# NikolasMarkou/blind_image_denoising

Measured on AMD Instinct MI355X. Metric: denoised images/sec (256x256x3) + MAE vs ref, resnet_1x18, higher is better.
Workload: dtype f16x2 split (hi+lo, fp32 accumulate)

## Files before the change

blind_image_denoising_amd/csrc/fused_h3w.hip:

```cpp
#include "h3v_core.h"
#include "h3_bands.h"
#include "base_rows.h"

#ifndef H3W_PRIO_SET
#define H3W_PRIO_SET 0
#endif
#if H3W_PRIO_SET == 1
#define H3W_PRIO_A1 0
#define H3W_PRIO_B1 1
#define H3W_PRIO_A2 2
#define H3W_PRIO_B2 3
#elif H3W_PRIO_SET == 2
#define H3W_PRIO_A1 3
#define H3W_PRIO_B1 2
#define H3W_PRIO_A2 1
#define H3W_PRIO_B2 0
#elif H3W_PRIO_SET == 3
#define H3W_PRIO_A1 0
#define H3W_PRIO_B1 2
#define H3W_PRIO_A2 0
#define H3W_PRIO_B2 2
#elif H3W_PRIO_SET == 4
#define H3W_PRIO_A1 2
#define H3W_PRIO_B1 0
#define H3W_PRIO_A2 2
#define H3W_PRIO_B2 0
#endif
#ifndef H3W_PRIO_A1
#define H3W_PRIO_A1 1
#endif
#ifndef H3W_PRIO_B1
#define H3W_PRIO_B1 1
#endif
#ifndef H3W_PRIO_A2
#define H3W_PRIO_A2 1
#endif
#ifndef H3W_PRIO_B2
#define H3W_PRIO_B2 1
#endif

#ifndef H3W_XCD_ORDER
#define H3W_XCD_ORDER 1
#endif

struct H3WGeom {
    static constexpr int NG = 9, GW = 16 * NG;
    static constexpr int G = 3;
    static constexpr int NR = 3, NW = 12, NT = 768;
    static constexpr int SW = 128;
    static constexpr int PITCH = (GW + 2) * 16;
    static constexpr int NRX0 = 5, NRM = 2, NRX1 = 3, NRO = 2;
    static constexpr int PD = 3;
    static constexpr int UNROLL = 6;
    static constexpr int X0_PLANE = (NRX0 * PITCH + 255) / 256 * 256, M_PLANE = (NRM * PITCH + 255) / 256 * 256;
    static constexpr int X1_PLANE = (NRX1 * PITCH + 255) / 256 * 256;
    static constexpr int OUT_PLANE = GW * 16, OUT_SLOT = 4 * OUT_PLANE;
    static constexpr int X0_OFF = 0, M1_OFF = X0_OFF + 4 * X0_PLANE, X1_OFF = M1_OFF + 4 * M_PLANE, M2_OFF = X1_OFF + 4 * X1_PLANE;
    static constexpr int OUT_OFF = M2_OFF + 4 * M_PLANE, LDS_BYTES = OUT_OFF + NRO * OUT_SLOT;
    static constexpr int BIN_RING = 4, BIN_ROWPX = GW + 4;
    static constexpr int BIN_SLOT = 2 * BIN_ROWPX * 8;
    static constexpr int BIN_OFF = LDS_BYTES, BWA_OFF = BIN_OFF + BIN_RING * BIN_SLOT, BINVS_OFF = BWA_OFF + 3 * 64 * 16;
    static constexpr int BRED_OFF = BINVS_OFF + 16, LDS_BYTES_BASE = BRED_OFF + NT * 4;
    static_assert(LDS_BYTES_BASE <= 160 * 1024 && BIN_OFF % 16 == 0 && BIN_SLOT % 16 == 0 && LDS_BYTES_BASE % 16 == 0, "LDS (producer)");
    static constexpr int LEAD = 12;
    static constexpr int NSTAMP = 4;
    static_assert(UNROLL % NRM == 0 && UNROLL % NRO == 0 && UNROLL % NRX1 == 0 && UNROLL % 3 == 0, "static slots");
    static_assert(NRX0 == PD + 2, "x0 ring: rows s-1 (residual), s (conv1a), s+1 (landed), s+2, s+3 (in flight)");
    static_assert(LDS_BYTES <= 160 * 1024, "LDS");
    static_assert(3 * X0_PLANE + NRX0 * PITCH < 65536, "fragment offsets fit the 16-bit ds offset");
};

struct H3WTile : BandUnit {
    int X0, X1;
    int G0;
    int D0, D1;
};

__device__ __forceinline__ H3WTile h3w_tile(const FusedH3WArgs& a, const int t)
{
    H3WTile r{bf_band_unit<H3W_XCD_ORDER != 0>(a, t)};
    r.X0 = r.sx * H3WGeom::SW;
    r.X1 = min(a.W, r.X0 + H3WGeom::SW);
    r.G0 = min(max(r.X0 - 8, 0), max(a.W - H3WGeom::GW, 0));
    r.D0 = max(0, (r.X0 - 4) & ~7);
    r.D1 = min(a.W, (r.X1 + 4 + 7) & ~7);
    return r;
}

template <int INP>
struct H3WRoleA {
    using Gm = H3WGeom;
    const char* tin;
    char* tmid;
    h8 w[13];
    f32x4 acc[Gm::G][3];
    int rp, rs;
    int wr;
    float inv_s, relu_floor;
    float lane_scale[Gm::G];
    bool skip_last = false;

    __device__ __forceinline__ void init(const void* wimg, const FusedH3WArgs& a, const float* aux, const int lane, const int gc0)
    {
        const int q = lane >> 4;
#pragma unroll
        for (int i = 0; i < 13; ++i) w[i] = reinterpret_cast<const h8*>(wimg)[bf_band_wimage(a, i) * 64 + lane];
        inv_s = aux[0];
        relu_floor = a.act1_relu ? 0.f : -__builtin_inff();
        rp = (q & 1) * INP + (gc0 + (q >> 1)) * 16;
        rs = ((q & 1) + 2 * (q >> 1)) * INP + (gc0 + 2) * 16;
        wr = (q >> 1) * Gm::M_PLANE + (gc0 + 1) * 16 + (q & 1) * 8;
#pragma unroll
        for (int g = 0; g < Gm::G; ++g)
#pragma unroll
            for (int k = 0; k < 3; ++k) acc[g][k] = (f32x4){0.f, 0.f, 0.f, 0.f};
    }
    __device__ __forceinline__ void set_tile(const H3WTile& t, const int W, const int gc0)
    {
#pragma unroll
        for (int g = 0; g < Gm::G; ++g) lane_scale[g] = (t.G0 + gc0 + 16 * g < W) ? inv_s : 0.f;
    }

    __device__ __forceinline__ H3VFrag load(const int islot_bytes, const int g) const
    {
        H3VFrag f;
        const char* p = tin + rp + islot_bytes;
        f.ph = *reinterpret_cast<const h8*>(p + g * 256);
        f.pl = *reinterpret_cast<const h8*>(p + g * 256 + 2 * INP);
        f.s = *reinterpret_cast<const h8*>(tin + rs + islot_bytes + g * 256);
        return f;
    }

    __device__ __forceinline__ H3VEpi<true> epilogue(const int g, const int mslot, const f32x4 v, const bool rowok) const
    {
        H3VEpi<true> e;
        e.v = v;
        e.sc = rowok ? lane_scale[g] : 0.f;
        e.floor_ = relu_floor;
        e.p = tmid + wr + mslot * Gm::PITCH + g * 256;
        e.lo_off = 2 * Gm::M_PLANE;
        return e;
    }

    template <int J, class Epi>
    __device__ __forceinline__ void mfmas(const int g, const int a1, const int a2, const H3VFrag& cur, f32x4& c0, Epi* epi)
    {
        if constexpr (J < 15) {
            constexpr int k = J / 3, which = J % 3;
            if (!(H3V_ABLATE & 8) && !(skip_last && g == Gm::G - 1)) {
                if constexpr (which == 0) acc[g][a2] = h3v_mfma(cur, w, 2, k, acc[g][a2]);
                else if constexpr (which == 1) acc[g][a1] = h3v_mfma(cur, w, 1, k, acc[g][a1]);
                else c0 = h3v_mfma(cur, w, 0, k, c0);
            } else if (J == 0) {
                acc[g][a2][0] += (float)cur.ph[0] + (float)cur.pl[1] + (float)cur.s[2];
            }
            __builtin_amdgcn_sched_barrier(0);
            if constexpr (J >= 2) {
                if (epi) epi->template pair<J - 2>();
            }
            mfmas<J + 1>(g, a1, a2, cur, c0, epi);
        }
    }

    template <int PH, class Hook>
    __device__ __forceinline__ void step(const int islot_bytes, const bool rowok, Hook& hook)
    {
        constexpr int a0 = PH % 3, a1 = (PH + 2) % 3, a2 = (PH + 1) % 3;
        constexpr int mslot = PH % Gm::NRM;
        H3VFrag cur = load(islot_bytes, 0);
#pragma unroll
        for (int g = 0; g < Gm::G; ++g) {
            H3VFrag nx;
            if (g + 1 < Gm::G) nx = load(islot_bytes, g + 1);
            __builtin_amdgcn_sched_barrier(0);
            f32x4 c0 = {0.f, 0.f, 0.f, 0.f};
            if (g > 0) {
                H3VEpi<true> e = epilogue(g - 1, mslot, acc[g - 1][a2], rowok);
                mfmas<0>(g, a1, a2, cur, c0, &e);
            } else {
                mfmas<0>(g, a1, a2, cur, c0, (H3VEpi<true>*)nullptr);
                hook.after_first_group();
                __builtin_amdgcn_sched_barrier(0);
            }
            acc[g][a0] = c0;
            if (g + 1 < Gm::G) cur = nx;
        }
        H3VEpi<true> e = epilogue(Gm::G - 1, mslot, bf_acc_ready(acc[Gm::G - 1][a2]), rowok);
        e.all();
    }
};

template <int RESP, int OUTP>
struct H3WRoleB {
    using Gm = H3WGeom;
    const char* tmid;
    const char* tres;
    char* tout;
    h8 w[13];
    f32x4 acc[Gm::G][3];
    int rp, rs;
    int rr;
    int wo;
    float inv_s2;
    f32x4 shs;
    float lane_scale[Gm::G];
    bool skip_last = false;

    __device__ __forceinline__ void init(const void* wimg, const FusedH3WArgs& a, const float* aux, const int lane, const int gc0,
                                         const bool out_is_ring)
    {
        const int q = lane >> 4;
#pragma unroll
        for (int i = 0; i < 13; ++i) w[i] = reinterpret_cast<const h8*>(wimg)[bf_band_wimage(a, i) * 64 + lane];
        inv_s2 = aux[48];
        shs = *reinterpret_cast<const f32x4*>(aux + 32 + q * 4) * (1.0f / inv_s2);
        rp = (q & 1) * Gm::M_PLANE + (gc0 + (q >> 1)) * 16;
        rs = ((q & 1) + 2 * (q >> 1)) * Gm::M_PLANE + (gc0 + 2) * 16;
        rr = ((q & 1) + 2 * (q >> 1)) * RESP + (gc0 + 1) * 16;
        wo = (q >> 1) * OUTP + (gc0 + (out_is_ring ? 1 : 0)) * 16 + (q & 1) * 8;
#pragma unroll
        for (int g = 0; g < Gm::G; ++g)
#pragma unroll
            for (int k = 0; k < 3; ++k) acc[g][k] = (f32x4){0.f, 0.f, 0.f, 0.f};
    }
    __device__ __forceinline__ void set_tile(const H3WTile& t, const int W, const int gc0)
    {
#pragma unroll
        for (int g = 0; g < Gm::G; ++g) lane_scale[g] = (t.G0 + gc0 + 16 * g < W) ? inv_s2 : 0.f;
    }

    __device__ __forceinline__ H3VFrag load(const int mslot, const int g) const
    {
        H3VFrag f;
        const int o = mslot * Gm::PITCH + g * 256;
        f.ph = *reinterpret_cast<const h8*>(tmid + rp + o);
        f.pl = *reinterpret_cast<const h8*>(tmid + rp + o + 2 * Gm::M_PLANE);
        f.s = *reinterpret_cast<const h8*>(tmid + rs + o);
        return f;
    }
    __device__ __forceinline__ h8 load_res(const int xslot_bytes, const int g) const
    {
        return *reinterpret_cast<const h8*>(tres + rr + xslot_bytes + g * 256);
    }

    __device__ __forceinline__ H3VEpi<false> epilogue(const int g, const int oslot_bytes, const f32x4 accv, const bool rowok) const
    {
        H3VEpi<false> e;
        e.v = accv;
        e.sc = rowok ? lane_scale[g] : 0.f;
        e.floor_ = 0.f;
        e.p = tout + wo + oslot_bytes + g * 256;
        e.lo_off = 2 * OUTP;
        return e;
    }

    template <int J, class Epi>
    __device__ __forceinline__ void mfmas(const int g, const int a1, const int a2, const H3VFrag& cur, const h8 xr, f32x4& c0, Epi* epi)
    {
        if constexpr (J < 16) {
            if (!(H3V_ABLATE & 4) && !(skip_last && g == Gm::G - 1)) {
                if constexpr (J == 0) {
                    c0 = MFMA_H(w[12], xr, shs);
                } else {
                    constexpr int k = (J - 1) / 3, which = (J - 1) % 3;
                    if constexpr (which == 0) acc[g][a2] = h3v_mfma(cur, w, 2, k, acc[g][a2]);
                    else if constexpr (which == 1) acc[g][a1] = h3v_mfma(cur, w, 1, k, acc[g][a1]);
                    else c0 = h3v_mfma(cur, w, 0, k, c0);
                }
            } else if (J == 0) {
                acc[g][a2][0] += (float)cur.ph[0] + (float)cur.pl[1] + (float)cur.s[2] + (float)xr[3];
            }
            __builtin_amdgcn_sched_barrier(0);
            if constexpr (J >= 2) {
                if (epi) epi->template pair<J - 2>();
            }
            mfmas<J + 1>(g, a1, a2, cur, xr, c0, epi);
        }
    }

    template <int PH, class Hook>
    __device__ __forceinline__ void step(const int xslot_bytes, const int oslot_bytes, const bool rowok, Hook& hook)
    {
        constexpr int mslot = (PH + 1) % Gm::NRM;
        constexpr int a0 = PH % 3, a1 = (PH + 2) % 3, a2 = (PH + 1) % 3;
        H3VFrag cur = load(mslot, 0);
        h8 xr = load_res(xslot_bytes, 0);
#pragma unroll
        for (int g = 0; g < Gm::G; ++g) {
            H3VFrag nx;
            h8 xn;
            if (g + 1 < Gm::G) {
                nx = load(mslot, g + 1);
                xn = load_res(xslot_bytes, g + 1);
            }
            __builtin_amdgcn_sched_barrier(0);
            f32x4 c0;
            if (g > 0) {
                H3VEpi<false> e = epilogue(g - 1, oslot_bytes, acc[g - 1][a2], rowok);
                mfmas<0>(g, a1, a2, cur, xr, c0, &e);
            } else {
                mfmas<0>(g, a1, a2, cur, xr, c0, (H3VEpi<false>*)nullptr);
                hook.after_first_group();
                __builtin_amdgcn_sched_barrier(0);
            }
            acc[g][a0] = c0;
            if (g + 1 < Gm::G) {
                cur = nx;
                xr = xn;
            }
        }
        H3VEpi<false> e = epilogue(Gm::G - 1, oslot_bytes, bf_acc_ready(acc[Gm::G - 1][a2]), rowok);
        e.all();
    }
};

#ifndef H3W_MEM_ROLES
#define H3W_MEM_ROLES 0
#endif
constexpr int h3w_mem_kind(const int role)
{
    constexpr int loader[4] = {2, 0, 1, 3}, storer[4] = {0, 1, 0, 0};
    return role == loader[H3W_MEM_ROLES] ? 1 : (role == storer[H3W_MEM_ROLES] ? 2 : 0);
}

template <int KIND>
struct H3WMem {
    __device__ __forceinline__ H3WMem(const FusedH3WArgs&, char*, const char*, int, unsigned) {}
    __device__ __forceinline__ void set_tile(const H3WTile&, int) {}
    __device__ __forceinline__ void prologue(const H3WTile&) {}
    __device__ __forceinline__ void begin(const H3WTile&, int, int) {}
    __device__ __forceinline__ void after_first_group() {}
    __device__ __forceinline__ void end() {}
    __device__ __forceinline__ void finish() {}
};

template <>
struct H3WMem<1> {
    using Gm = H3WGeom;
    const FusedH3WArgs& a;
    char* tin;
    int piece;
    unsigned plane_g;
    unsigned col_off;
    bool active;
    int dslot;

    __device__ __forceinline__ H3WMem(const FusedH3WArgs& a_, char* tx0, const char*, const int rw, const unsigned pg)
        : a(a_), tin(tx0), piece(rw), plane_g(pg), col_off(0), active(false), dslot(0) {}
    __device__ __forceinline__ void set_tile(const H3WTile& t, const int lane)
    {
        const int c = t.G0 + 64 * piece + lane;
        active = (c >= t.D0) & (c < t.D1) & (64 * piece + lane < Gm::GW);
        col_off = (unsigned)c * 16u;
    }
    __device__ __forceinline__ void dma_row(const H3WTile& t, const int r, const int slot) const
    {
        if (H3V_ABLATE & 1) return;
        const int y = t.y(r - 4);
        const bool ok = (y >= 0) & (y < a.H) & (r < t.nrows + 8);
#pragma unroll
        for (int plane = 0; plane < 4; ++plane) {
            const char* src = ok ? reinterpret_cast<const char*>(a.in) + t.img + (size_t)plane * plane_g + (size_t)y * a.W * 16 + col_off
                                 : reinterpret_cast<const char*>(a.zeros);
            char* dst = tin + plane * Gm::X0_PLANE + slot * Gm::PITCH + (1 + 64 * piece) * 16;
            if (active) h3_dma16(src, dst);
        }
    }
    static constexpr int INFLIGHT = 2 * 4;
    __device__ __forceinline__ void wait_landed() const { __builtin_amdgcn_s_waitcnt(h3_vmcnt((H3V_ABLATE & 1) ? 0 : INFLIGHT)); }
    __device__ __forceinline__ void prologue(const H3WTile& t)
    {
#pragma unroll
        for (int r = 0; r < Gm::PD; ++r) dma_row(t, r, r);
        wait_landed();
        dslot = Gm::PD;
    }
    __device__ __forceinline__ void begin(const H3WTile& t, const int s, int)
    {
        dma_row(t, s + Gm::PD, dslot);
        dslot = h3v_wrap(dslot + 1, Gm::NRX0);
    }
    __device__ __forceinline__ void after_first_group() {}
    __device__ __forceinline__ void end() { wait_landed(); }
    __device__ __forceinline__ void finish() { __builtin_amdgcn_s_waitcnt(h3_vmcnt(0)); }
};

template <>
struct H3WMem<2> {
    using Gm = H3WGeom;
    const FusedH3WArgs& a;
    const char* tout;
    int first, np;
    unsigned plane_g;
    int st_off[3];
    unsigned g_off[3];
    bool okc[3];
    h8 rec[3];
    bool have;
    char* image;
    size_t row_off;

    __device__ __forceinline__ H3WMem(const FusedH3WArgs& a_, char*, const char* tout_, const int rw, const unsigned pg)
        : a(a_), tout(tout_), first(3 * rw), np(rw < 2 ? 3 : 2), plane_g(pg), have(false), image(nullptr), row_off(0) {}
    __device__ __forceinline__ void set_tile(const H3WTile& t, const int lane)
    {
#pragma unroll
        for (int i = 0; i < 3; ++i) {
            const int p = first + i, plane = p >> 1, c = t.X0 + 64 * (p & 1) + lane;
            okc[i] = (i < np) & (c < t.X1);
            st_off[i] = plane * Gm::OUT_PLANE + (c - t.G0) * 16;
            g_off[i] = (unsigned)plane * plane_g + (unsigned)c * 16u;
        }
    }
    __device__ __forceinline__ void prologue(const H3WTile&) {}
    __device__ __forceinline__ void begin(const H3WTile& t, const int s, const int PH)
    {
        const int k = s - Gm::LEAD, oslot = (PH + 1) % Gm::NRO;
        have = (k >= 0) & (k < t.nrows) & !(H3V_ABLATE & 2);
        if (!have) return;
        image = reinterpret_cast<char*>(a.out) + t.img;
        row_off = (size_t)t.y(k) * a.W * 16;
#pragma unroll
        for (int i = 0; i < 3; ++i)
            if (i < np) rec[i] = *reinterpret_cast<const h8*>(tout + oslot * Gm::OUT_SLOT + st_off[i]);
    }
    __device__ __forceinline__ void after_first_group()
    {
        if (!have) return;
#pragma unroll
        for (int i = 0; i < 3; ++i)
            if (okc[i]) h3_stream_store16(image, 4u * plane_g, row_off, g_off[i], rec[i]);
    }
    __device__ __forceinline__ void end() {}
    __device__ __forceinline__ void finish() {}
};

template <>
struct H3WMem<3> {
    using Gm = H3WGeom;
    const FusedH3WArgs& a;
    const char* tout;
    int half;
    int st_off;
    int col;
    bool okc;

    __device__ __forceinline__ H3WMem(const FusedH3WArgs& a_, char*, const char* tout_, const int rw, const unsigned)
        : a(a_), tout(tout_), half(rw), st_off(0), col(0), okc(false) {}
    __device__ __forceinline__ void set_tile(const H3WTile& t, const int lane)
    {
        col = t.X0 + 64 * half + lane;
        okc = (half < 2) & (col < t.X1) & (col < a.Wo);
        st_off = (col - t.G0) * 16;
    }
    __device__ __forceinline__ void prologue(const H3WTile&) {}
    __device__ __forceinline__ void begin(const H3WTile& t, const int s, const int PH)
    {
        const int k = s - Gm::LEAD, oslot = (PH + 1) % Gm::NRO;
        bool have = (half < 2) & (k >= 0) & (k < t.nrows) & !(H3V_ABLATE & 2);
        if (have) have = t.y(k) < a.Ho;
        if (!have) return;
        char* orow = reinterpret_cast<char*>(a.head_out) + ((size_t)t.b * a.Ho + (size_t)t.y(k)) * a.Wo * 3 * (a.head_u8 ? 1 : 4);
        const char* src = tout + oslot * Gm::OUT_SLOT + st_off;
        float h0 = 0.f, h1 = 0.f, h2 = 0.f;
#pragma unroll
        for (int hf = 0; hf < 2; ++hf) {
            const h8 hi = *reinterpret_cast<const h8*>(src + hf * Gm::OUT_PLANE), lo = *reinterpret_cast<const h8*>(src + (2 + hf) * Gm::OUT_PLANE);
#pragma unroll
            for (int c = 0; c < 8; ++c) {
                const float v = (float)hi[c] + (float)lo[c];
                const f32x4 w = *reinterpret_cast<const f32x4*>(a.head_wh + (hf * 8 + c) * 4);
                h0 = fmaf(v, w.x, h0);
                h1 = fmaf(v, w.y, h1);
                h2 = fmaf(v, w.z, h2);
            }
        }
        const bool finite = fabsf(h0) <= 3.0e38f && fabsf(h1) <= 3.0e38f && fabsf(h2) <= 3.0e38f;
        if (!finite && a.status) atomicOr(a.status, BF_STATUS_F16_RANGE);
        float r[3] = {h0, h1, h2};
#pragma unroll
        for (int o = 0; o < 3; ++o) {
            float v = (1.0f - 2.0f / (__expf(4.0f * r[o]) + 1.0f)) * 0.51f;
            if (a.denormalize) v = (fminf(fmaxf(v, -0.5f), 0.5f) + 0.5f) * (a.v_max - a.v_min) + a.v_min;
            r[o] = v;
        }
        if (!okc) return;
        if (a.head_u8) {
            unsigned char* p = reinterpret_cast<unsigned char*>(orow) + (size_t)col * 3;
#pragma unroll
            for (int o = 0; o < 3; ++o) p[o] = (unsigned char)fminf(fmaxf(rintf(r[o]), 0.f), 255.f);
        } else {
            float* p = reinterpret_cast<float*>(orow) + (size_t)col * 3;
#pragma unroll
            for (int o = 0; o < 3; ++o) p[o] = r[o];
        }
        __builtin_amdgcn_sched_barrier(0);
    }
    __device__ __forceinline__ void after_first_group() {}
    __device__ __forceinline__ void end() {}
    __device__ __forceinline__ void finish() {}
};

#ifndef H3W_BASE_SPREAD
#define H3W_BASE_SPREAD 1
#endif
constexpr int h3w_base_groups(const int role)
{
    return H3W_BASE_SPREAD == 0 ? (role == 2 ? 3 : 0) : (H3W_BASE_SPREAD == 1 ? (role >= 1 ? 1 : 0) : (role <= 2 ? 1 : 0));
}
constexpr int h3w_base_first_group(const int role, const int rw)
{
    return H3W_BASE_SPREAD == 0 ? 3 * rw : (H3W_BASE_SPREAD == 1 ? 3 * (role - 1) + rw : 3 * role + rw);
}
constexpr bool h3w_base_fetches(const int role) { return role == 2; }

template <int NGW, bool FETCH>
struct H3WProducer {
    using Gm = H3WGeom;
    const FusedH3WArgs& a;
    char* tx0;
    char* tring;
    const char* twa;
    int g0, fw;
    float inv_s, floor_;
    int wr;
    int fo;
    int col0;
    int px, xcol;
    const uint8_t* img;
    unsigned raw[3];
    BrPixel rawp;
    int dslot;

    __device__ __forceinline__ H3WProducer(const FusedH3WArgs& a_, char* lds, const int g0_, const int fw_)
        : a(a_), tx0(lds + Gm::X0_OFF), tring(lds + Gm::BIN_OFF), twa(lds + Gm::BWA_OFF), g0(g0_), fw(fw_), wr(0), fo(0), col0(0),
          px(0), xcol(0), img(nullptr), raw{0u, 0u, 0u}, rawp{false, false}, dslot(0)
    {
        inv_s = *reinterpret_cast<const float*>(lds + Gm::BINVS_OFF);
        floor_ = a.base_relu ? 0.f : -__builtin_inff();
    }
    __device__ __forceinline__ void set_tile(const H3WTile& t, const int lane)
    {
        const int n = lane & 15, q = lane >> 4, gc0 = 16 * g0 + n;
        wr = (q >> 1) * Gm::X0_PLANE + (gc0 + 1) * 16 + (q & 1) * 8;
        const int p = gc0 + 2 * (q & 1);
        fo = ((p & 1) * Gm::BIN_ROWPX + (p & ~1)) * 8;
        twa = tx0 - Gm::X0_OFF + Gm::BWA_OFF + lane * 16;
        col0 = t.G0 + gc0;
        px = 64 * fw + lane;
        xcol = t.G0 - 1 + px;
        img = reinterpret_cast<const uint8_t*>(a.base_u8) + (size_t)t.b * a.Hs * a.Ws * 3;
    }
    __device__ __forceinline__ void request(const H3WTile& t, const int u)
    {
        const int yy = t.ybase + u - 5;
        const bool need = (px < Gm::GW + 2) & (u <= t.nrows + 9);
        rawp = br_pixel(yy, xcol, a.H, a.W, a.Hs, a.Ws);
        rawp.inside &= need;
        rawp.colour &= need;
        if (rawp.colour) {
            const uint8_t* p = img + ((size_t)yy * a.Ws + xcol) * 3;
            raw[0] = p[0];
            raw[1] = p[1];
            raw[2] = p[2];
        }
    }
    __device__ __forceinline__ void commit(const int u)
    {
        if (px >= Gm::GW + 2) return;
        const h4 v = br_record(rawp, raw[0], raw[1], raw[2]);
        h4* row = reinterpret_cast<h4*>(tring + (u & (Gm::BIN_RING - 1)) * Gm::BIN_SLOT);
        row[px] = v;
        if (px > 0) row[Gm::BIN_ROWPX + px - 1] = v;
    }
    __device__ __forceinline__ void produce(const H3WTile& t, const int r, const int slot)
    {
        if (r >= t.nrows + 8) return;
        const int y = t.y(r - 4);
        const bool rowok = (y >= 0) & (y < a.H);
        f32x4 acc[NGW];
#pragma unroll
        for (int g = 0; g < NGW; ++g) acc[g] = (f32x4){0.f, 0.f, 0.f, 0.f};
#pragma unroll
        for (int dy = 0; dy < 3; ++dy) {
            const h8 wa = *reinterpret_cast<const h8*>(twa + dy * 64 * 16);
            const char* row = tring + ((r + dy) & (Gm::BIN_RING - 1)) * Gm::BIN_SLOT + fo;
#pragma unroll
            for (int g = 0; g < NGW; ++g) acc[g] = MFMA_H(wa, *reinterpret_cast<const h8*>(row + g * 128), acc[g]);
        }
#pragma unroll
        for (int g = 0; g < NGW; ++g) {
            H3VEpi<true> e;
            e.v = bf_acc_ready(acc[g]);
            e.sc = (rowok & (col0 + 16 * g < a.W)) ? inv_s : 0.f;
            e.floor_ = floor_;
            e.p = tx0 + wr + slot * Gm::PITCH + g * 256;
            e.lo_off = 2 * Gm::X0_PLANE;
            e.all();
        }
    }
    __device__ __forceinline__ void fill(const H3WTile& t)
    {
        if constexpr (FETCH) {
#pragma unroll
            for (int u = 0; u < Gm::BIN_RING; ++u) {
                request(t, u);
                commit(u);
            }
            request(t, Gm::BIN_RING);
        }
    }
    __device__ __forceinline__ void prologue(const H3WTile& t)
    {
        produce(t, 0, 0);
        dslot = 1;
    }
    __device__ __forceinline__ void begin(const H3WTile& t, const int s)
    {
        if constexpr (FETCH) {
            commit(s + 4);
            request(t, s + 5);
        }
        produce(t, s + 1, dslot);
        dslot = h3v_wrap(dslot + 1, Gm::NRX0);
        __builtin_amdgcn_sched_barrier(0);
    }
};

template <>
struct H3WProducer<0, false> {
    __device__ __forceinline__ H3WProducer(const FusedH3WArgs&, char*, int, int) {}
    __device__ __forceinline__ void set_tile(const H3WTile&, int) {}
    __device__ __forceinline__ void fill(const H3WTile&) {}
    __device__ __forceinline__ void prologue(const H3WTile&) {}
    __device__ __forceinline__ void begin(const H3WTile&, int) {}
};

template <bool HEAD, bool BASE>
constexpr int h3w_hook_kind(const int role)
{
    const int k = h3w_mem_kind(role);
    return (HEAD && k == 2) ? 3 : ((BASE && k == 1) ? 0 : k);
}

template <bool HEAD, bool BASE>
__global__ __launch_bounds__(H3WGeom::NT, 3) void fused_block2_h3w_kernel(FusedH3WArgs a)
{
    using Gm = H3WGeom;
    extern __shared__ __attribute__((aligned(16))) char h3w_lds[];
    char* tx0 = h3w_lds + Gm::X0_OFF;
    char* tm1 = h3w_lds + Gm::M1_OFF;
    char* tx1 = h3w_lds + Gm::X1_OFF;
    char* tm2 = h3w_lds + Gm::M2_OFF;
    char* tout = h3w_lds + Gm::OUT_OFF;
    const int tid = threadIdx.x, lane = tid & 63;
    const int wave = __builtin_amdgcn_readfirstlane(tid >> 6);
    const int n = lane & 15;
    const int role = wave / Gm::NR, rw = wave - role * Gm::NR;
    const unsigned plane_g = (unsigned)a.H * (unsigned)a.W * 16u;
    const int gc0 = 16 * Gm::G * rw + n;

    if (BASE && a.status && blockIdx.x == 0 && tid == 0) *a.status = 0;
    for (int i = tid * 16; i < (BASE ? Gm::LDS_BYTES_BASE : Gm::LDS_BYTES); i += Gm::NT * 16)
        *reinterpret_cast<f32x4*>(h3w_lds + i) = (f32x4){0.f, 0.f, 0.f, 0.f};
    __syncthreads();
    if constexpr (BASE) {
        const float bs = br_weight_scale(a.base_w, reinterpret_cast<float*>(h3w_lds + Gm::BRED_OFF));
        if (wave == 0) {
#pragma unroll
            for (int dy = 0; dy < 3; ++dy)
                *reinterpret_cast<h8*>(h3w_lds + Gm::BWA_OFF + (dy * 64 + lane) * 16) = br_operand(a.base_w, bs, dy, lane);
            if (lane == 0) *reinterpret_cast<float*>(h3w_lds + Gm::BINVS_OFF) = 1.0f / bs;
        }
        __syncthreads();
    }

#if H3V_ABLATE & 32
    unsigned long long stamp_sum[Gm::NSTAMP] = {0, 0, 0, 0}, stamp_prev, real0;
    asm volatile("s_memrealtime %0\n\ts_memtime %1\n\ts_waitcnt lgkmcnt(0)" : "=s"(real0), "=s"(stamp_prev)::"memory");
#endif

#define H3W_ROW_IN_IMAGE(k) ((t.y(k) >= 0) & (t.y(k) < a.H))
#define H3W_BAND(R, M, P, ACTIVE, STEP)                                                                         \
    for (int ti = blockIdx.x; ti < a.ntiles; ti += gridDim.x) {                                               \
        const H3WTile t = h3w_tile(a, ti);                                                                    \
        R.set_tile(t, a.W, gc0);                                                                              \
        M.set_tile(t, lane);                                                                                  \
        P.set_tile(t, lane);                                                                                  \
        if constexpr (BASE) {                                      \
            P.fill(t);                                                                                        \
            h3v_barrier();                                                                                    \
        }                                                                                                     \
        P.prologue(t);                                                                                        \
        M.prologue(t);                                                                                        \
        h3v_barrier();                                                 \
        const int nsteps = t.nrows + Gm::LEAD;                                                                \
        int slot5 = 0;                                                                           \
        for (int s0 = 0; s0 < nsteps; s0 += Gm::UNROLL) {                                                     \
            H3W_ONE(0, M, P, ACTIVE, STEP); H3W_ONE(1, M, P, ACTIVE, STEP); H3W_ONE(2, M, P, ACTIVE, STEP);   \
            H3W_ONE(3, M, P, ACTIVE, STEP); H3W_ONE(4, M, P, ACTIVE, STEP); H3W_ONE(5, M, P, ACTIVE, STEP);   \
        }                                                                                                     \
        M.finish();                                                                                           \
        h3v_barrier();                                                                                        \
    }
#define H3W_ONE(PH, M, P, ACTIVE, STEP)                                                                         \
    do {                                                                                                      \
        const int s = s0 + PH;                                                                                \
        P.begin(t, s);                                                                                        \
        M.begin(t, s, PH);                                                                                    \
        if (ACTIVE(s)) { STEP(PH); }                                                                          \
        else M.after_first_group();                                                                           \
        slot5 = h3v_wrap(slot5 + 1, Gm::NRX0);                                                                \
        H3V_STAMP(0);                                                                                         \
        M.end();                                                                                              \
        H3V_STAMP(1);                                                                                         \
        h3v_barrier();                                                                                        \
        H3V_STAMP(2);                                                                                         \
    } while (0)

    if (role == 0) {
        __builtin_amdgcn_s_setprio(H3W_PRIO_A1);
        H3WRoleA<Gm::X0_PLANE> R;
        R.tin = tx0; R.tmid = tm1;
        R.init(a.w1r[0], a, a.aux[0], lane, gc0);
        R.skip_last = (H3V_ABLATE & 256) && rw == Gm::NR - 1;
        H3WMem<h3w_hook_kind<HEAD, BASE>(0)> M(a, tx0, tout, rw, plane_g);
        H3WProducer<BASE ? h3w_base_groups(0) : 0, BASE && h3w_base_groups(0) && h3w_base_fetches(0)> P(a, h3w_lds, h3w_base_first_group(0, rw), rw);
        __builtin_amdgcn_s_waitcnt(h3_vmcnt(0));
#define H3W_ACTIVE(s) ((s) < t.nrows + 8)
#define H3W_STEP(PH) R.template step<PH>(slot5 * Gm::PITCH, (s >= 2) & H3W_ROW_IN_IMAGE(s - 5), M)
        H3W_BAND(R, M, P, H3W_ACTIVE, H3W_STEP)
#undef H3W_ACTIVE
#undef H3W_STEP
    } else if (role == 1) {
        __builtin_amdgcn_s_setprio(H3W_PRIO_B1);
        H3WRoleB<Gm::X0_PLANE, Gm::X1_PLANE> R;
        R.tmid = tm1; R.tres = tx0; R.tout = tx1;
        R.init(a.w2r[0], a, a.aux[0], lane, gc0, true);
        R.skip_last = (H3V_ABLATE & 256) && rw == Gm::NR - 1;
        H3WMem<h3w_hook_kind<HEAD, BASE>(1)> M(a, tx0, tout, rw, plane_g);
        H3WProducer<BASE ? h3w_base_groups(1) : 0, BASE && h3w_base_groups(1) && h3w_base_fetches(1)> P(a, h3w_lds, h3w_base_first_group(1, rw), rw);
        __builtin_amdgcn_s_waitcnt(h3_vmcnt(0));
#define H3W_ACTIVE(s) (((s) >= 3) & ((s) < t.nrows + 9))
#define H3W_STEP(PH) R.template step<PH>(h3v_wrap(slot5 + Gm::NRX0 - 1, Gm::NRX0) * Gm::PITCH, (PH % Gm::NRX1) * Gm::PITCH, H3W_ROW_IN_IMAGE(s - 7), M)
        H3W_BAND(R, M, P, H3W_ACTIVE, H3W_STEP)
#undef H3W_ACTIVE
#undef H3W_STEP
    } else if (role == 2) {
        __builtin_amdgcn_s_setprio(H3W_PRIO_A2);
        H3WRoleA<Gm::X1_PLANE> R;
        R.tin = tx1; R.tmid = tm2;
        R.init(a.w1r[1], a, a.aux[1], lane, gc0);
        R.skip_last = (H3V_ABLATE & 256) && rw == Gm::NR - 1;
        H3WMem<h3w_hook_kind<HEAD, BASE>(2)> M(a, tx0, tout, rw, plane_g);
        H3WProducer<BASE ? h3w_base_groups(2) : 0, BASE && h3w_base_groups(2) && h3w_base_fetches(2)> P(a, h3w_lds, h3w_base_first_group(2, rw), rw);
        __builtin_amdgcn_s_waitcnt(h3_vmcnt(0));
#define H3W_ACTIVE(s) (((s) >= 6) & ((s) < t.nrows + 10))
#define H3W_STEP(PH) R.template step<PH>(((PH + 2) % Gm::NRX1) * Gm::PITCH, H3W_ROW_IN_IMAGE(s - 9), M)
        H3W_BAND(R, M, P, H3W_ACTIVE, H3W_STEP)
#undef H3W_ACTIVE
#undef H3W_STEP
    } else {
        __builtin_amdgcn_s_setprio(H3W_PRIO_B2);
        H3WRoleB<Gm::X1_PLANE, Gm::OUT_PLANE> R;
        R.tmid = tm2; R.tres = tx1; R.tout = tout;
        R.init(a.w2r[1], a, a.aux[1], lane, gc0, false);
        R.skip_last = (H3V_ABLATE & 256) && rw == Gm::NR - 1;
        H3WMem<h3w_hook_kind<HEAD, BASE>(3)> M(a, tx0, tout, rw, plane_g);
        H3WProducer<BASE ? h3w_base_groups(3) : 0, BASE && h3w_base_groups(3) && h3w_base_fetches(3)> P(a, h3w_lds, h3w_base_first_group(3, rw), rw);
        __builtin_amdgcn_s_waitcnt(h3_vmcnt(0));
#define H3W_ACTIVE(s) (((s) >= 9) & ((s) < t.nrows + 11))
#define H3W_STEP(PH) R.template step<PH>(((PH + 1) % Gm::NRX1) * Gm::PITCH, (PH % Gm::NRO) * Gm::OUT_SLOT, true, M)
        H3W_BAND(R, M, P, H3W_ACTIVE, H3W_STEP)
#undef H3W_ACTIVE
#undef H3W_STEP
    }
#undef H3W_BAND
#undef H3W_ONE
#undef H3W_ROW_IN_IMAGE
#if H3V_ABLATE & 32
    {
        unsigned long long real1;
        asm volatile("s_memrealtime %0\n\ts_waitcnt lgkmcnt(0)" : "=s"(real1)::"memory");
        stamp_sum[3] = real1 - real0;
    }
    if (a.dbg && lane == 0) {
        for (int k = 0; k < Gm::NSTAMP; ++k) a.dbg[((size_t)blockIdx.x * Gm::NW + wave) * 8 + k] = stamp_sum[k];
    }
#endif
}

bool bf_fused_block2_h3w_supports(int H, int W) { return W >= 1 && H >= 1; }

hipError_t bf_launch_fused_block2_h3w(const FusedH3WArgs& args, hipStream_t s)
{
    using Gm = H3WGeom;
    FusedH3WArgs a = args;
    if (!a.zeros || (!a.in && !a.base_u8) || (!a.out && !a.head_wh) || !bf_fused_block2_h3w_supports(a.H, a.W)) return hipErrorInvalidValue;
    if (a.base_u8 && (!a.base_w || a.head_wh || a.reverse_tiles || a.Hs < 1 || a.Ws < 1 || a.Hs > a.H || a.Ws > a.W)) return hipErrorInvalidValue;
    if ((int64_t)a.H * a.W * 64 >= ((int64_t)1 << 32)) return hipErrorInvalidValue;
    const BandPlan p = bf_band_plan(a.B, a.H, (a.W + Gm::SW - 1) / Gm::SW, Gm::LEAD + 2);
    a.nstrips = p.nstrips;
    a.rows_per_tile = p.rows_per_tile;
    a.tiles_y = p.tiles_y;
    a.ntiles = p.ntiles;
    if (a.head_wh && (!a.head_out || a.Ho < 1 || a.Wo < 1 || a.Ho > a.H || a.Wo > a.W)) return hipErrorInvalidValue;
    void (*kernel)(FusedH3WArgs) = a.base_u8 ? fused_block2_h3w_kernel<false, true>
                                   : a.head_wh ? fused_block2_h3w_kernel<true, false> : fused_block2_h3w_kernel<false, false>;
    const int lds = a.base_u8 ? Gm::LDS_BYTES_BASE : Gm::LDS_BYTES;
    const hipError_t e = bf_set_max_lds(reinterpret_cast<const void*>(kernel), lds);
    if (e != hipSuccess) return e;
    hipLaunchKernelGGL(kernel, dim3(p.grid), dim3(Gm::NT), lds, s, a);
    return hipGetLastError();
}
```

blind_image_denoising_amd/csrc/h3v_core.h:

```cpp
#pragma once
#include "bf_common.h"
#include "h3_core.h"

#ifndef H3V_ABLATE
#define H3V_ABLATE 0
#endif
#ifndef H3_LOAD_POLICY
#define H3_LOAD_POLICY 2
#endif
#ifndef H3_STORE_POLICY
#define H3_STORE_POLICY 16
#endif
static_assert((H3_LOAD_POLICY & ~18) == 0 && (H3_STORE_POLICY & ~18) == 0, "aux bits: 2 = nt, 16 = sc1");
#ifndef H3V_PRIO_B
#define H3V_PRIO_B 1
#endif
#ifndef H3V_PRIO_MODE
#define H3V_PRIO_MODE 0
#endif

struct H3VFrag {
    h8 ph, pl, s;
};

__device__ __forceinline__ f32x4 h3v_mfma(const H3VFrag& x, const h8 (&w)[13], const int dy, const int m, f32x4 acc)
{
    switch (m) {
        case 0: return MFMA_H(w[dy * 4 + 0], x.ph, acc);
        case 1: return MFMA_H(w[dy * 4 + 1], x.ph, acc);
        case 2: return MFMA_H(w[dy * 4 + 0], x.pl, acc);
        case 3: return MFMA_H(w[dy * 4 + 2], x.s, acc);
        default: return MFMA_H(w[dy * 4 + 3], x.s, acc);
    }
}

__device__ __forceinline__ void h3v_barrier()
{
#if H3V_ABLATE & 16
    __builtin_amdgcn_s_waitcnt(H3_LGKMCNT0);
    asm volatile("" ::: "memory");
#else
    h3_barrier();
#endif
}

#if H3V_ABLATE & 32
#define H3V_STAMP(k)                                                                                     \
    do {                                                                                                 \
        unsigned long long now_;                                                                         \
        __builtin_amdgcn_sched_barrier(0);                                                               \
        asm volatile("s_memtime %0\n\ts_waitcnt lgkmcnt(0)" : "=s"(now_)::"memory");                      \
        __builtin_amdgcn_sched_barrier(0);                                                               \
        stamp_sum[k] += now_ - stamp_prev;                                                               \
        stamp_prev = now_;                                                                               \
    } while (0)
#else
#define H3V_STAMP(k) do { } while (0)
#endif

__device__ __forceinline__ int h3v_wrap(const int v, const int n) { return v >= n ? v - n : v; }

__device__ __forceinline__ void h3_dma16(const char* src, char* dst)
{
    __builtin_amdgcn_global_load_lds((const __attribute__((address_space(1))) void*)src, (__attribute__((address_space(3))) void*)dst,
                                     16, 0, H3_LOAD_POLICY);
}

__device__ __forceinline__ h8 h3_stream_load16(const char* src)
{
    if constexpr (H3_LOAD_POLICY & 2) return __builtin_nontemporal_load(reinterpret_cast<const h8*>(src));
    else return *reinterpret_cast<const h8*>(src);
}

__device__ __forceinline__ void h3_stream_store16(char* image, const unsigned image_bytes, const size_t row_off, const unsigned lane_off, const h8 v)
{
    if constexpr (H3_STORE_POLICY == 0) {
        *reinterpret_cast<h8*>(image + row_off + lane_off) = v;
    } else if constexpr (H3_STORE_POLICY == 2) {
        __builtin_nontemporal_store(v, reinterpret_cast<h8*>(image + row_off + lane_off));
    } else {
        typedef unsigned h3_u4 __attribute__((ext_vector_type(4)));
        const __amdgpu_buffer_rsrc_t rsrc = __builtin_amdgcn_make_buffer_rsrc(image, 0, (int)image_bytes, 0x00020000);
        __builtin_amdgcn_raw_buffer_store_b128(__builtin_bit_cast(h3_u4, v), rsrc, (int)lane_off, (int)row_off, H3_STORE_POLICY);
    }
}

typedef unsigned h3v_u2 __attribute__((ext_vector_type(2)));
template <bool RELU>
struct H3VEpi {
    static constexpr int NOPS = (RELU ? 4 : 0) + 10;
    f32x4 v;
    float sc, floor_;
    unsigned h0, h1, l0, l1;
    char* p;
    int lo_off;
    template <int I> __device__ __forceinline__ void op()
    {
        constexpr int K = RELU ? I - 4 : I;
        if constexpr (RELU && I < 4) {
            if (!(H3V_ABLATE & 64)) {
                float r;
                asm volatile("v_max_f32 %0, %1, %2" : "=v"(r) : "v"(v[I]), "v"(floor_));
                v[I] = r;
            }
        } else if constexpr (K == 0) asm volatile("v_fma_mixlo_f16 %0, %1, %2, 0" : "=v"(h0) : "v"(v.x), "v"(sc));
        else if constexpr (K == 1) asm volatile("v_fma_mixlo_f16 %0, %1, %2, 0" : "=v"(h1) : "v"(v.z), "v"(sc));
        else if constexpr (K == 2) asm volatile("v_fma_mixhi_f16 %0, %1, %2, 0" : "+v"(h0) : "v"(v.y), "v"(sc));
        else if constexpr (K == 3) asm volatile("v_fma_mixhi_f16 %0, %1, %2, 0" : "+v"(h1) : "v"(v.w), "v"(sc));
        else if constexpr (K == 4) asm volatile("v_fma_mixlo_f16 %0, %1, %2, -%3 op_sel_hi:[0,0,1]" : "=v"(l0) : "v"(v.x), "v"(sc), "v"(h0));
        else if constexpr (K == 5) asm volatile("v_fma_mixlo_f16 %0, %1, %2, -%3 op_sel_hi:[0,0,1]" : "=v"(l1) : "v"(v.z), "v"(sc), "v"(h1));
        else if constexpr (K == 6) asm volatile("v_fma_mixhi_f16 %0, %1, %2, -%3 op_sel:[0,0,1] op_sel_hi:[0,0,1]" : "+v"(l0) : "v"(v.y), "v"(sc), "v"(h0));
        else if constexpr (K == 7) asm volatile("v_fma_mixhi_f16 %0, %1, %2, -%3 op_sel:[0,0,1] op_sel_hi:[0,0,1]" : "+v"(l1) : "v"(v.w), "v"(sc), "v"(h1));
        else if constexpr (K == 8) *reinterpret_cast<h3v_u2*>(p) = (H3V_ABLATE & 64) ? (h3v_u2){__builtin_bit_cast(unsigned, v.x), __builtin_bit_cast(unsigned, v.y)} : (h3v_u2){h0, h1};
        else if constexpr (K == 9) *reinterpret_cast<h3v_u2*>(p + lo_off) = (H3V_ABLATE & 64) ? (h3v_u2){__builtin_bit_cast(unsigned, v.z), __builtin_bit_cast(unsigned, v.w)} : (h3v_u2){l0, l1};
        __builtin_amdgcn_sched_barrier(0);
    }
    template <int SLOT> __device__ __forceinline__ void pair()
    {
        if constexpr (2 * SLOT < NOPS) op<2 * SLOT>();
        if constexpr (2 * SLOT + 1 < NOPS) op<2 * SLOT + 1>();
    }
    template <int I = 0> __device__ __forceinline__ void all()
    {
        if constexpr (I < NOPS) {
            op<I>();
            all<I + 1>();
        }
    }
};
```

Measured before the change: 30610.

## Store RoleB epilogue outputs directly to global memory, bypassing LDS staging ring

```diff
diff --git a/blind_image_denoising_amd/csrc/fused_h3w.hip b/blind_image_denoising_amd/csrc/fused_h3w.hip
--- a/blind_image_denoising_amd/csrc/fused_h3w.hip
+++ b/blind_image_denoising_amd/csrc/fused_h3w.hip
@@ -43,6 +43,10 @@
 #define H3W_XCD_ORDER 1
 #endif
 
+#ifndef H3W_DIRECT_STORE
+#define H3W_DIRECT_STORE 1
+#endif
+
 struct H3WGeom {
     static constexpr int NG = 9, GW = 16 * NG;
     static constexpr int G = 3;
@@ -56,7 +60,8 @@
     static constexpr int X1_PLANE = (NRX1 * PITCH + 255) / 256 * 256;
     static constexpr int OUT_PLANE = GW * 16, OUT_SLOT = 4 * OUT_PLANE;
     static constexpr int X0_OFF = 0, M1_OFF = X0_OFF + 4 * X0_PLANE, X1_OFF = M1_OFF + 4 * M_PLANE, M2_OFF = X1_OFF + 4 * X1_PLANE;
-    static constexpr int OUT_OFF = M2_OFF + 4 * M_PLANE, LDS_BYTES = OUT_OFF + NRO * OUT_SLOT;
+    static constexpr int OUT_OFF = M2_OFF + 4 * M_PLANE, LDS_BYTES_STAGED = OUT_OFF + NRO * OUT_SLOT;
+    static constexpr int LDS_BYTES = H3W_DIRECT_STORE ? OUT_OFF : LDS_BYTES_STAGED;
     static constexpr int BIN_RING = 4, BIN_ROWPX = GW + 4;
     static constexpr int BIN_SLOT = 2 * BIN_ROWPX * 8;
     static constexpr int BIN_OFF = LDS_BYTES, BWA_OFF = BIN_OFF + BIN_RING * BIN_SLOT, BINVS_OFF = BWA_OFF + 3 * 64 * 16;
@@ -66,7 +71,7 @@
     static constexpr int NSTAMP = 4;
     static_assert(UNROLL % NRM == 0 && UNROLL % NRO == 0 && UNROLL % NRX1 == 0 && UNROLL % 3 == 0, "static slots");
     static_assert(NRX0 == PD + 2, "x0 ring: rows s-1 (residual), s (conv1a), s+1 (landed), s+2, s+3 (in flight)");
-    static_assert(LDS_BYTES <= 160 * 1024, "LDS");
+    static_assert(LDS_BYTES_STAGED <= 160 * 1024 && LDS_BYTES <= LDS_BYTES_STAGED && LDS_BYTES % 16 == 0 && LDS_BYTES_STAGED % 16 == 0, "LDS");
     static_assert(3 * X0_PLANE + NRX0 * PITCH < 65536, "fragment offsets fit the 16-bit ds offset");
 };
 
@@ -190,9 +195,36 @@
     }
 };
 
-template <int RESP, int OUTP>
+struct H3WEpiStore : H3VEpi<false> {
+    char* image;
+    unsigned image_bytes, off;
+    size_t row_hi, row_lo;
+    unsigned long long mask;
+    __device__ __forceinline__ void store()
+    {
+        if (__builtin_amdgcn_inverse_ballot_w64(mask)) {
+            h3_stream_store8(image, image_bytes, row_hi, off, (H3V_ABLATE & 64) ? (h3v_u2){__builtin_bit_cast(unsigned, v.x), __builtin_bit_cast(unsigned, v.y)} : (h3v_u2){h0, h1});
+            h3_stream_store8(image, image_bytes, row_lo, off, (H3V_ABLATE & 64) ? (h3v_u2){__builtin_bit_cast(unsigned, v.z), __builtin_bit_cast(unsigned, v.w)} : (h3v_u2){l0, l1});
+        }
+        __builtin_amdgcn_sched_barrier(0);
+    }
+    template <int SLOT> __device__ __forceinline__ void pair()
+    {
+        if constexpr (SLOT < 4) H3VEpi<false>::template pair<SLOT>();
+        else if constexpr (SLOT == 4) store();
+    }
+    __device__ __forceinline__ void all()
+    {
+        pair<0>(); pair<1>(); pair<2>(); pair<3>(); pair<4>();
+    }
+};
+template <bool DIRECT> struct H3WEpiOf { using type = H3VEpi<false>; };
+template <> struct H3WEpiOf<true> { using type = H3WEpiStore; };
+
+template <int RESP, int OUTP, bool DIRECT = false>
 struct H3WRoleB {
     using Gm = H3WGeom;
+    using Epi = typename H3WEpiOf<DIRECT>::type;
     const char* tmid;
     const char* tres;
     char* tout;
@@ -205,11 +237,26 @@
     f32x4 shs;
     float lane_scale[Gm::G];
     bool skip_last = false;
+    char* gout;
+    char* image;
+    unsigned plane_g;
+    unsigned go;
+    unsigned long long okm[Gm::G];
+    bool have;
+    size_t row_hi, row_lo;
 
     __device__ __forceinline__ void init(const void* wimg, const FusedH3WArgs& a, const float* aux, const int lane, const int gc0,
                                          const bool out_is_ring)
     {
         const int q = lane >> 4;
+        gout = reinterpret_cast<char*>(a.out);
+        plane_g = (unsigned)a.H * (unsigned)a.W * 16u;
+        image = nullptr;
+        go = 0;
+        have = false;
+        row_hi = row_lo = 0;
+#pragma unroll
+        for (int g = 0; g < Gm::G; ++g) okm[g] = 0;
 #pragma unroll
         for (int i = 0; i < 13; ++i) w[i] = reinterpret_cast<const h8*>(wimg)[bf_band_wimage(a, i) * 64 + lane];
         inv_s2 = aux[48];
@@ -227,6 +274,21 @@
     {
 #pragma unroll
         for (int g = 0; g < Gm::G; ++g) lane_scale[g] = (t.G0 + gc0 + 16 * g < W) ? inv_s2 : 0.f;
+        if constexpr (DIRECT) {
+            const int q = (threadIdx.x & 63) >> 4, c0 = t.G0 + gc0;
+#pragma unroll
+            for (int g = 0; g < Gm::G; ++g) okm[g] = __builtin_amdgcn_ballot_w64((c0 + 16 * g >= t.X0) & (c0 + 16 * g < t.X1));
+            go = (unsigned)(q >> 1) * plane_g + (unsigned)c0 * 16u + (unsigned)(q & 1) * 8u;
+            image = gout + t.img;
+        }
+    }
+    __device__ __forceinline__ void set_row(const H3WTile& t, const int W, const int k)
+    {
+        if constexpr (DIRECT) {
+            have = (k >= 0) & (k < t.nrows) & !(H3V_ABLATE & 2);
+            row_hi = (size_t)t.y(have ? k : 0) * W * 16;
+            row_lo = row_hi + 2 * (size_t)plane_g;
+        }
     }
 
     __device__ __forceinline__ H3VFrag load(const int mslot, const int g) const
@@ -243,14 +305,25 @@
         return *reinterpret_cast<const h8*>(tres + rr + xslot_bytes + g * 256);
     }
 
-    __device__ __forceinline__ H3VEpi<false> epilogue(const int g, const int oslot_bytes, const f32x4 accv, const bool rowok) const
-    {
-        H3VEpi<false> e;
+    __device__ __forceinline__ Epi epilogue(const int g, const int oslot_bytes, const f32x4 accv, const bool rowok) const
+    {
+        Epi e;
         e.v = accv;
         e.sc = rowok ? lane_scale[g] : 0.f;
         e.floor_ = 0.f;
-        e.p = tout + wo + oslot_bytes + g * 256;
-        e.lo_off = 2 * OUTP;
+        if constexpr (DIRECT) {
+            e.p = nullptr;
+            e.lo_off = 0;
+            e.image = image;
+            e.image_bytes = 4u * plane_g;
+            e.off = go + 256u * g;
+            e.row_hi = row_hi;
+            e.row_lo = row_lo;
+            e.mask = have ? okm[g] : 0ull;
+        } else {
+            e.p = tout + wo + oslot_bytes + g * 256;
+            e.lo_off = 2 * OUTP;
+        }
         return e;
     }
 
@@ -296,10 +369,10 @@
             __builtin_amdgcn_sched_barrier(0);
             f32x4 c0;
             if (g > 0) {
-                H3VEpi<false> e = epilogue(g - 1, oslot_bytes, acc[g - 1][a2], rowok);
+                Epi e = epilogue(g - 1, oslot_bytes, acc[g - 1][a2], rowok);
                 mfmas<0>(g, a1, a2, cur, xr, c0, &e);
             } else {
-                mfmas<0>(g, a1, a2, cur, xr, c0, (H3VEpi<false>*)nullptr);
+                mfmas<0>(g, a1, a2, cur, xr, c0, (Epi*)nullptr);
                 hook.after_first_group();
                 __builtin_amdgcn_sched_barrier(0);
             }
@@ -309,7 +382,7 @@
                 xr = xn;
             }
         }
-        H3VEpi<false> e = epilogue(Gm::G - 1, oslot_bytes, bf_acc_ready(acc[Gm::G - 1][a2]), rowok);
+        Epi e = epilogue(Gm::G - 1, oslot_bytes, bf_acc_ready(acc[Gm::G - 1][a2]), rowok);
         e.all();
     }
 };
@@ -317,6 +390,7 @@
 #ifndef H3W_MEM_ROLES
 #define H3W_MEM_ROLES 0
 #endif
+static_assert(!(H3W_DIRECT_STORE && H3W_MEM_ROLES == 3), "loads and stores on different waves");
 constexpr int h3w_mem_kind(const int role)
 {
     constexpr int loader[4] = {2, 0, 1, 3}, storer[4] = {0, 1, 0, 0};
@@ -636,11 +710,13 @@
     __device__ __forceinline__ void begin(const H3WTile&, int) {}
 };
 
+template <bool HEAD>
+constexpr bool h3w_direct() { return H3W_DIRECT_STORE != 0 && !HEAD; }
 template <bool HEAD, bool BASE>
 constexpr int h3w_hook_kind(const int role)
 {
     const int k = h3w_mem_kind(role);
-    return (HEAD && k == 2) ? 3 : ((BASE && k == 1) ? 0 : k);
+    return k == 2 ? (HEAD ? 3 : (h3w_direct<HEAD>() ? 0 : 2)) : ((BASE && k == 1) ? 0 : k);
 }
 
 template <bool HEAD, bool BASE>
@@ -652,7 +728,9 @@
     char* tm1 = h3w_lds + Gm::M1_OFF;
     char* tx1 = h3w_lds + Gm::X1_OFF;
     char* tm2 = h3w_lds + Gm::M2_OFF;
-    char* tout = h3w_lds + Gm::OUT_OFF;
+    constexpr bool DIRECT = h3w_direct<HEAD>();
+    constexpr int LDS_RINGS = DIRECT ? Gm::LDS_BYTES : Gm::LDS_BYTES_STAGED;
+    char* tout = DIRECT ? nullptr : h3w_lds + Gm::OUT_OFF;
     const int tid = threadIdx.x, lane = tid & 63;
     const int wave = __builtin_amdgcn_readfirstlane(tid >> 6);
     const int n = lane & 15;
@@ -661,7 +739,7 @@
     const int gc0 = 16 * Gm::G * rw + n;
 
     if (BASE && a.status && blockIdx.x == 0 && tid == 0) *a.status = 0;
-    for (int i = tid * 16; i < (BASE ? Gm::LDS_BYTES_BASE : Gm::LDS_BYTES); i += Gm::NT * 16)
+    for (int i = tid * 16; i < (BASE ? Gm::LDS_BYTES_BASE : LDS_RINGS); i += Gm::NT * 16)
         *reinterpret_cast<f32x4*>(h3w_lds + i) = (f32x4){0.f, 0.f, 0.f, 0.f};
     __syncthreads();
     if constexpr (BASE) {
@@ -762,7 +840,7 @@
 #undef H3W_STEP
     } else {
         __builtin_amdgcn_s_setprio(H3W_PRIO_B2);
-        H3WRoleB<Gm::X1_PLANE, Gm::OUT_PLANE> R;
+        H3WRoleB<Gm::X1_PLANE, Gm::OUT_PLANE, DIRECT> R;
         R.tmid = tm2; R.tres = tx1; R.tout = tout;
         R.init(a.w2r[1], a, a.aux[1], lane, gc0, false);
         R.skip_last = (H3V_ABLATE & 256) && rw == Gm::NR - 1;
@@ -770,7 +848,7 @@
         H3WProducer<BASE ? h3w_base_groups(3) : 0, BASE && h3w_base_groups(3) && h3w_base_fetches(3)> P(a, h3w_lds, h3w_base_first_group(3, rw), rw);
         __builtin_amdgcn_s_waitcnt(h3_vmcnt(0));
 #define H3W_ACTIVE(s) (((s) >= 9) & ((s) < t.nrows + 11))
-#define H3W_STEP(PH) R.template step<PH>(((PH + 1) % Gm::NRX1) * Gm::PITCH, (PH % Gm::NRO) * Gm::OUT_SLOT, true, M)
+#define H3W_STEP(PH) R.set_row(t, a.W, s - (Gm::LEAD - 1)); R.template step<PH>(((PH + 1) % Gm::NRX1) * Gm::PITCH, (PH % Gm::NRO) * Gm::OUT_SLOT, true, M)
         H3W_BAND(R, M, P, H3W_ACTIVE, H3W_STEP)
 #undef H3W_ACTIVE
 #undef H3W_STEP
@@ -807,7 +885,7 @@
     if (a.head_wh && (!a.head_out || a.Ho < 1 || a.Wo < 1 || a.Ho > a.H || a.Wo > a.W)) return hipErrorInvalidValue;
     void (*kernel)(FusedH3WArgs) = a.base_u8 ? fused_block2_h3w_kernel<false, true>
                                    : a.head_wh ? fused_block2_h3w_kernel<true, false> : fused_block2_h3w_kernel<false, false>;
-    const int lds = a.base_u8 ? Gm::LDS_BYTES_BASE : Gm::LDS_BYTES;
+    const int lds = a.base_u8 ? Gm::LDS_BYTES_BASE : (a.head_wh ? Gm::LDS_BYTES_STAGED : Gm::LDS_BYTES);
     const hipError_t e = bf_set_max_lds(reinterpret_cast<const void*>(kernel), lds);
     if (e != hipSuccess) return e;
     hipLaunchKernelGGL(kernel, dim3(p.grid), dim3(Gm::NT), lds, s, a);
diff --git a/blind_image_denoising_amd/csrc/h3v_core.h b/blind_image_denoising_amd/csrc/h3v_core.h
--- a/blind_image_denoising_amd/csrc/h3v_core.h
+++ b/blind_image_denoising_amd/csrc/h3v_core.h
@@ -86,6 +86,18 @@
 }
 
 typedef unsigned h3v_u2 __attribute__((ext_vector_type(2)));
+__device__ __forceinline__ void h3_stream_store8(char* image, const unsigned image_bytes, const size_t row_off, const unsigned lane_off, const h3v_u2 v)
+{
+    if constexpr (H3_STORE_POLICY == 0) {
+        *reinterpret_cast<h3v_u2*>(image + row_off + lane_off) = v;
+    } else if constexpr (H3_STORE_POLICY == 2) {
+        __builtin_nontemporal_store(v, reinterpret_cast<h3v_u2*>(image + row_off + lane_off));
+    } else {
+        const __amdgpu_buffer_rsrc_t rsrc = __builtin_amdgcn_make_buffer_rsrc(image, 0, (int)image_bytes, 0x00020000);
+        __builtin_amdgcn_raw_buffer_store_b64(v, rsrc, (int)lane_off, (int)row_off, H3_STORE_POLICY);
+    }
+}
+
 template <bool RELU>
 struct H3VEpi {
     static constexpr int NOPS = (RELU ? 4 : 0) + 10;
```

After: 31180, median of 6. +1.9%, better.
